# xiph/daala

Hardware: AMD Instinct MI355X
Metric: 1080p all-intra transform blocks/s (filter+DCT+PVQ) (higher is better)
Workload: dtype int32 (lifting DCT/filters) + f64 (PVQ search)

## Files before the change

### daala_amd/csrc/od_occupancy.cuh

```cuda
#pragma once
#ifndef ODHIP_SEARCH_OCC
# define ODHIP_SEARCH_OCC 0
#endif
#if ODHIP_SEARCH_OCC == 2
# define OD_SEARCH_OCC_ATTR __attribute__((amdgpu_waves_per_eu(2), amdgpu_num_vgpr(100)))
# define OD_SEARCH_VGPR_FLOOR() asm volatile("" ::: "v175")
#elif ODHIP_SEARCH_OCC == 3
# define OD_SEARCH_OCC_ATTR __attribute__((amdgpu_waves_per_eu(3), amdgpu_num_vgpr(68)))
# define OD_SEARCH_VGPR_FLOOR() asm volatile("" ::: "v128")
#else
# define OD_SEARCH_OCC_ATTR __attribute__((amdgpu_waves_per_eu(3)))
# define OD_DECIDE_OCC_ATTR
# define OD_SEARCH_VGPR_FLOOR() ((void)0)
#endif
#ifndef OD_DECIDE_OCC_ATTR
# define OD_DECIDE_OCC_ATTR OD_SEARCH_OCC_ATTR
#endif
#ifndef ODHIP_SEARCH_WAVES
# define ODHIP_SEARCH_WAVES 1
#endif
```

### daala_amd/csrc/pvq_lane.cuh

```cuda
#pragma once
#include "od_sel.cuh"

namespace {

constexpr int kPitch = 64;
constexpr int kRsqN = 512;

__device__ double gRsqTable[kRsqN];

__global__ void k_rsq_fill(void) {
  const int i = threadIdx.x;
  if (i < kRsqN) {
    gRsqTable[i] = i < 16 ? kRsqrtTable[i] : __ddiv_rn(1., __dsqrt_rn((double)(i + 1)));
  }
}

struct LaneSearch {
  double xx;
  double norm2;
  double l1_inv;
  unsigned xmax;
  unsigned xy;
  unsigned yy;
  int i;
// ... 74 lines not shown
  unsigned xmax = 0;
#pragma unroll 8
  for (int j = 0; j < N; j++) {
    const unsigned ax = pk[j*kPitch + lane] >> 16;
    xx += (unsigned long long)ax*ax;
    l1 += ax;
    xmax = ax > xmax ? ax : xmax;
  }
  xx = od_grp_add<S>(xx);
  l1 = od_grp_add<S>(l1);
  xmax = od_grp_umax<S>(xmax);
  s.xx = (double)xx;
  s.norm2 = 2*__ddiv_rn(1., __dsqrt_rn(1e-30 + s.xx));
  const double l1d = (double)l1;
  s.l1_inv = __ddiv_rn(1., l1d > 1e-100 ? l1d : 1e-100);
  s.xmax = xmax;
  s.xy = 0;
  s.yy = 0;
  s.i = 0;
}

constexpr int kGrp = 8;

template <int N>
__device__ __forceinline__ void od_lane_load_group(uint32_t (&w)[kGrp], const uint32_t *pk, int lane,
 int g) {
#pragma unroll
  for (int t = 0; t < kGrp; t++) {
    const int j = g*kGrp + t;
    w[t] = j < N ? pk[j*kPitch + lane] : 0;
  }
}

template <int N, bool ACCEL>
__device__ __forceinline__ int od_lane_rdo_scan(const uint32_t *pk, const double *rsq, int lane,
 unsigned xy, unsigned base, double norm2, double lambda, double delta_rate, double accel_rate,
 int jbase, double &best_out) {
  if (N <= 16) {
    double best = 0;
    int pos = jbase;
    int jv = jbase;
#pragma unroll 4
    for (int j = 0; j < N; j++) {
      const uint32_t w = pk[j*kPitch + lane];
      const double tt = (double)(xy + (w >> 16));
      const double r = rsq[base + (w & 0xffffu)];
      if (j > 0) od_inc(jv);
      const double jd = (double)jv;
      const double val = (tt*norm2)*r - (lambda*jd)*(ACCEL ? delta_rate + jd*accel_rate : delta_rate);
      if (j == 0) best = val;
      else {
        const unsigned long long m = od_cmp_gt(val, best);
        best = od_sel(m, val, best);
        pos = od_sel(m, jv, pos);
      }
    }
    best_out = best;
    return pos;
  }
  constexpr int NG = (N + kGrp - 1)/kGrp;
  uint32_t w0[kGrp];
  uint32_t w1[kGrp];
  uint32_t w2[kGrp];
  double r0[kGrp];
  double r1[kGrp];
  od_lane_load_group<N>(w0, pk, lane, 0);
  od_lane_load_group<N>(w1, pk, lane, 1);
#pragma unroll
  for (int t = 0; t < kGrp; t++) r0[t] = rsq[base + (w0[t] & 0xffffu)];
  double best = 0;
  int pos = jbase;
  int jv = jbase;
#pragma unroll
  for (int g = 0; g < NG; g++) {
    if (g + 2 < NG) od_lane_load_group<N>(w2, pk, lane, g + 2);
    if (g + 1 < NG) {
#pragma unroll
      for (int t = 0; t < kGrp; t++) r1[t] = rsq[base + (w1[t] & 0xffffu)];
    }
    __builtin_amdgcn_sched_barrier(0);
#pragma unroll
    for (int t = 0; t < kGrp; t++) {
      const int j = g*kGrp + t;
      if (j < N) {
        const double tt = (double)(xy + (w0[t] >> 16));
        if (j > 0) od_inc(jv);
        const double jd = (double)jv;
        const double val = (tt*norm2)*r0[t]
         - (lambda*jd)*(ACCEL ? delta_rate + jd*accel_rate : delta_rate);
        if (j == 0) best = val;
        else {
          const unsigned long long m = od_cmp_gt(val, best);
          best = od_sel(m, val, best);
          pos = od_sel(m, jv, pos);
        }
      }
    }
    __builtin_amdgcn_sched_barrier(0);
#pragma unroll
    for (int t = 0; t < kGrp; t++) {
      w0[t] = w1[t];
      w1[t] = w2[t];
      r0[t] = r1[t];
    }
  }
  best_out = best;
  return pos;
}

template <int N>
__device__ __forceinline__ int od_lane_greedy_scan(const uint32_t *pk, int lane, unsigned xy,
 unsigned yyp1, int jbase, double &ba_out, double &bb_out) {
  if (N <= 16) {
    double ba = 0;
    double bb = 1;
    int pos = jbase;
    int jv = jbase;
#pragma unroll 4
    for (int j = 0; j < N; j++) {
      const uint32_t w = pk[j*kPitch + lane];
      const double tt = (double)(xy + (w >> 16));
      const double a = tt*tt;
      const double b = (double)(yyp1 + (w & 0xffffu));
      if (j == 0) {
        ba = a;
        bb = b;
      }
      else {
        od_inc(jv);
        const unsigned long long m = od_cmp_gt(a*bb, ba*b);
        ba = od_sel(m, a, ba);
        bb = od_sel(m, b, bb);
        pos = od_sel(m, jv, pos);
      }
    }
    ba_out = ba;
    bb_out = bb;
    return pos;
  }
  constexpr int NG = (N + kGrp - 1)/kGrp;
  uint32_t w0[kGrp];
  uint32_t w1[kGrp];
  od_lane_load_group<N>(w0, pk, lane, 0);
  double ba = 0;
  double bb = 1;
  int pos = jbase;
  int jv = jbase;
#pragma unroll
  for (int g = 0; g < NG; g++) {
    if (g + 1 < NG) od_lane_load_group<N>(w1, pk, lane, g + 1);
    __builtin_amdgcn_sched_barrier(0);
#pragma unroll
    for (int t = 0; t < kGrp; t++) {
      const int j = g*kGrp + t;
      if (j < N) {
        const double tt = (double)(xy + (w0[t] >> 16));
        const double a = tt*tt;
        const double b = (double)(yyp1 + (w0[t] & 0xffffu));
        if (j == 0) {
          ba = a;
          bb = b;
        }
        else {
          od_inc(jv);
          const unsigned long long m = od_cmp_gt(a*bb, ba*b);
          ba = od_sel(m, a, ba);
          bb = od_sel(m, b, bb);
          pos = od_sel(m, jv, pos);
        }
      }
    }
    __builtin_amdgcn_sched_barrier(0);
#pragma unroll
    for (int t = 0; t < kGrp; t++) w0[t] = w1[t];
  }
  ba_out = ba;
  bb_out = bb;
  return pos;
}

#ifndef ODHIP_GREEDY_FRONTS
# define ODHIP_GREEDY_FRONTS 1
#endif
#ifndef ODHIP_FRONT_CLASSES
# define ODHIP_FRONT_CLASSES 8
#endif
#ifndef ODHIP_FRONT_MIN
# define ODHIP_FRONT_MIN 4
#endif
constexpr int kFrontClasses = ODHIP_FRONT_CLASSES;
constexpr int kFrontMinPulses = ODHIP_FRONT_MIN;

template <int N>
__device__ __forceinline__ uint32_t od_lane_front_scan(const uint32_t *pk, int lane, uint32_t c2) {
  static_assert(N % kGrp == 0, "whole groups");
  constexpr int NG = N/kGrp;
  uint32_t best = 0;
  uint32_t w0[kGrp];
// ... 68 lines not shown
    const double oa = od_pair_swap(ba);
    const double ob = od_pair_swap(bb);
    const int op = od_pair_swap(bpos);
    const int oc = od_pair_swap(bc);
    const bool ohave = od_pair_swap((int)have) != 0;
    const double l = oa*bb;
    const double r = ba*ob;
    const bool other = ohave && (!have || l > r || (l == r && op < bpos));
    const int pos = other ? op : bpos;
    const int cw = other ? oc : bc;
    const bool owner = pos/N == half;
    const int local = pos - jbase;
    uint32_t w = 0;
    if (step && owner) w = pk[local*kPitch + lane];
    w = od_grp_or<2>(w);
    const bool mine = step && owner;
    if (step) {
      s.xy += w >> 16;
      s.yy += (w & 0xffffu) + 1;
      if (owner) pk[local*kPitch + lane] = w + 2;
      s.i++;
    }
    const uint32_t nf = od_lane_front_scan<N>(pk, lane, mine ? 2u*(uint32_t)cw : 0xffffffffu);
    const uint32_t wkey = ((w + 2) & 0xffff0000u) + (0x10000u + (uint32_t)(N - 1 - local));
#pragma unroll
    for (int c = 0; c < kFrontClasses; c++) {
      if (mine && c == cw) fr[c] = nf;
      if (mine && c == cw + 1) fr[c] = wkey > fr[c] ? wkey : fr[c];
    }
    if (__any(mine && cw + 1 >= kFrontClasses)) return;
  }
}

template <int N, int S>
__device__ __forceinline__ double od_lane_search(LaneSearch &s, uint32_t *pk, const double *rsq,
 int lane, int half, bool on, bool fresh, int k, double g2, double pvq_norm_lambda,
 bool force_seq) {
  constexpr int NBAND = N*S;
  static_assert(S == 1 || S == 2 || S == 4, "one lane, a pair or a quad per band");
  const int jbase = S > 1 ? half*N : 0;
  fresh = fresh && on;
  if (__any(fresh)) {
    const double kd = fresh && k > 2 ? (double)k : 0.;
    unsigned xy = 0;
    unsigned yy = 0;
    int i = 0;
#pragma unroll 4
    for (int j = 0; j < N; j++) {
      const unsigned ax = pk[j*kPitch + lane] >> 16;
      const double tmp = (kd*(double)ax)*s.l1_inv;
      int yj = (int)floor(tmp);
      yj = yj > 0 ? yj : 0;
      if (fresh) pk[j*kPitch + lane] = ax << 16 | (unsigned)yj << 1;
      xy += ax*(unsigned)yj;
      yy += (unsigned)yj*(unsigned)yj;
      i += yj;
    }
    xy = od_grp_add<S>(xy);
    yy = od_grp_add<S>(yy);
    i = od_grp_add<S>(i);
    if (fresh) {
      s.xy = xy;
      s.yy = yy;
      s.i = i;
    }
  }
  const int rdo_pulses = 1 + k/4;
  const int n_greedy = k - rdo_pulses;
#if ODHIP_GREEDY_FRONTS
  if constexpr (S == 2 && N >= 32 && N % kGrp == 0) {
    if (!force_seq && __any(on && n_greedy - s.i >= kFrontMinPulses)) {
      od_lane_greedy_fronts<N>(s, pk, lane, half & 1, on, k, n_greedy);
    }
  }
#endif
  while (__any(on && s.i < n_greedy)) {
    const bool step = on && s.i < n_greedy;
    double ba;
    double bb;
    int pos = od_lane_greedy_scan<N>(pk, lane, s.xy, s.yy + 1, jbase, ba, bb);
    if constexpr (S > 1) {
      const double tmax = (double)(s.xy + s.xmax);
      const bool exact = !force_seq
       && (tmax*tmax)*(double)(s.yy + 2*(unsigned)k + 1) < 4503599627370496.;
      if (__any(step && !exact)) {
        double ra = od_grp_bcast<S, 0>(ba);
        double rb = od_grp_bcast<S, 0>(bb);
        int rp = od_grp_bcast<S, 0>(pos);
        auto rescan = [&](double &xa, double &xb, int &xp) {
#pragma unroll 1
          for (int j = 0; j < N; j++) {
            const uint32_t w = pk[j*kPitch + lane];
            const double tt = (double)(s.xy + (w >> 16));
            const double a = tt*tt;
            const double b = (double)(s.yy + 1 + (w & 0xffffu));
            if (a*xb > xa*b) {
              xa = a;
              xb = b;
              xp = jbase + j;
            }
          }
        };
        {
          double ta = ra;
          double tb = rb;
          int tp = rp;
          rescan(ta, tb, tp);
          ra = od_grp_bcast<S, 1>(ta);
          rb = od_grp_bcast<S, 1>(tb);
          rp = od_grp_bcast<S, 1>(tp);
        }
        if constexpr (S == 4) {
          double ta = ra;
          double tb = rb;
          int tp = rp;
          rescan(ta, tb, tp);
          ra = od_grp_bcast<4, 2>(ta);
          rb = od_grp_bcast<4, 2>(tb);
          rp = od_grp_bcast<4, 2>(tp);
          ta = ra;
          tb = rb;
          tp = rp;
          rescan(ta, tb, tp);
          rp = od_grp_bcast<4, 3>(tp);
        }
        pos = rp;
      }
      else {
        {
// ... 14 lines not shown
        }
        if constexpr (S == 4) {
          const double oa = od_quad_swap2(ba);
          const double ob = od_quad_swap2(bb);
          const int op = od_quad_swap2(pos);
          const bool up = (half & 2) != 0;
          const double la = up ? oa : ba;
          const double lb = up ? ob : bb;
          const int lp = up ? op : pos;
          const double xa = up ? ba : oa;
          const double xb = up ? bb : ob;
          const int xp = up ? pos : op;
          pos = xa*lb > la*xb ? xp : lp;
        }
      }
    }
    int owner = 1;
    int local = pos;
    if constexpr (S > 1) {
      owner = pos/N == half;
      local = pos - jbase;
    }
    uint32_t w = 0;
    if (step && owner) w = pk[local*kPitch + lane];
    w = od_grp_or<S>(w);
    if (step) {
      s.xy += w >> 16;
      s.yy += (w & 0xffffu) + 1;
      if (owner) pk[local*kPitch + lane] = w + 2;
      s.i++;
    }
  }
  const double lambda = __ddiv_rn(pvq_norm_lambda, 1e-30 + g2);
  double delta_rate = 3./NBAND;
  double accel_rate = 0.;
  if (k == 1) {
    if (NBAND == 15) {
      accel_rate = -8./NBAND;
      delta_rate = 4.5/NBAND - accel_rate;
    }
    else if (NBAND == 8) {
      accel_rate = 5.7/NBAND;
      delta_rate = 9.3/NBAND - accel_rate;
    }
  }
  while (__any(on && s.i < k)) {
    const bool step = on && s.i < k;
    int pos = 0;
    double best = 0;
    if (!__any(step && s.yy + 2*(unsigned)k + 1 > (unsigned)kRsqN)) {
      const unsigned base = step ? s.yy : 0;
      const unsigned xy = step ? s.xy : 0;
      if ((NBAND == 8 || NBAND == 15) && __any(step && k == 1)) {
        pos = od_lane_rdo_scan<N, true>(pk, rsq, lane, xy, base, s.norm2, lambda, delta_rate,
         accel_rate, jbase, best);
      }
      else {
        pos = od_lane_rdo_scan<N, false>(pk, rsq, lane, xy, base, s.norm2, lambda, delta_rate,
         accel_rate, jbase, best);
      }
    }
    else {
#pragma unroll 1
      for (int j = 0; j < N; j++) {
        const uint32_t w = pk[j*kPitch + lane];
        const double t = (double)(s.xy + (w >> 16));
        const unsigned idx = s.yy + (w & 0xffffu) + 1;
        double r;
        if (step && idx <= (unsigned)kRsqN) r = rsq[idx - 1];
        else r = od_rsqrt_beyond((int)(idx ? idx : 1));
        const int jg = jbase + j;
        const double val = (t*s.norm2)*r - (lambda*jg)*(delta_rate + jg*accel_rate);
        if (j == 0 || val > best) {
          best = val;
          pos = jg;
        }
      }
    }
    if constexpr (S > 1) {
      {
        const double ob = od_pair_swap(best);
        const int op = od_pair_swap(pos);
        const bool up = (half & 1) != 0;
        const double va = up ? ob : best;
        const double vb = up ? best : ob;
        const int pa = up ? op : pos;
        const int pb = up ? pos : op;
        const bool win = vb > va;
        best = win ? vb : va;
        pos = win ? pb : pa;
      }
      if constexpr (S == 4) {
        const double ob = od_quad_swap2(best);
        const int op = od_quad_swap2(pos);
        const bool up = (half & 2) != 0;
        const double va = up ? ob : best;
        const double vb = up ? best : ob;
        const int pa = up ? op : pos;
        const int pb = up ? pos : op;
        pos = vb > va ? pb : pa;
      }
    }
    int owner = 1;
    int local = pos;
    if constexpr (S > 1) {
      owner = pos/N == half;
// ... 17 lines not shown
```

### daala_amd/csrc/pvq_refbands.hip

```cpp
#include "../../include/daala_hip.h"
#include <math.h>
#include <stdio.h>
#include <stdlib.h>
#include <string.h>
#include "od_ctx.cuh"
#include "od_pvq_math.cuh"
#include "od_occupancy.cuh"
#include "od_krange.cuh"
#include "od_band_stage.cuh"
#include "gen/od_scan_tables.h"
#define OD_RSQ_TABLE_N 512
#define OD_RSQ_HUGE
#include "pvq_search.cuh"
#include "pvq_row.cuh"
#include "pvq_regs.cuh"

namespace {

constexpr int kMaxJobs = 8;
constexpr int kMaxItems = kMaxJobs*ODHIP_MAX_BANDS;
constexpr int kSlots = ODHIP_PVQ_REF_SLOTS;
constexpr int kUncCap = 1 << 16;
constexpr double kDefaultMargin = 1e-9;

struct RJob {
  const od_coeff *coef;
  const od_coeff *ref;
  const int16_t *qm;
  const int16_t *qm_inv;
  odhip_pvq_refband *rec;
  void *items;
  int16_t *y;
  int16_t *r16;
  int16_t *x16;
  int16_t *xr;
  const double *rate;
  int32_t *choice;
  od_coeff *dq;
  unsigned short *keys;
  unsigned *ids;
  unsigned *krange;
  long nblocks;
  int nplanes;
  int w;
  int h;
  int bs;
  int nb_bands;
  int len;
// ... 1271 lines not shown
      ax[i] = abs(t);
      sg |= (unsigned)(t < 0) << i;
      y[i] = 0;
    }
    if (pad) {
      ax[N - 1] = 0;
      sg &= ~(1u << (N - 1));
    }
    od_regs_norm<N>(ax, &xx, &norm_1);
  }
  __device__ __forceinline__ double search(int n_true, int k, int prev_k, double g2, double lambda) {
    return od_pvq_search_regs<N>(ax, y, n_true, k, prev_k, g2, lambda, xx, norm_1, &cxy, &cyy);
  }
  __device__ __forceinline__ int moment() const {
    int m = 0;
#pragma unroll
    for (int i = 1; i < N; i++) m += i*y[i];
    return m;
  }
  __device__ __forceinline__ void store(int16_t *dst) {
    uint4 *p = reinterpret_cast<uint4 *>(dst - SH);
    int t[N + SH];
    if (SH) t[0] = 0;
#pragma unroll
    for (int i = 0; i < N; i++) t[i + SH] = (sg >> i) & 1 ? -y[i] : y[i];
#pragma unroll
    for (int q = 0; q < (N + SH)/8; q++) {
      p[q] = make_uint4(pack16(t[8*q], t[8*q + 1]), pack16(t[8*q + 2], t[8*q + 3]),
       pack16(t[8*q + 4], t[8*q + 5]), pack16(t[8*q + 6], t[8*q + 7]));
    }
  }
};



__device__ __forceinline__ int neg_interleave(int x, int ref) {
  if (x < ref) return -2*(x - ref) - 1;
  if (x < 2*ref) return 2*(x - ref);
  return x - 1;
}

__device__ unsigned char gRBandOf[OD_SCAN_LEN];

template <int N, class YGet>
__device__ __forceinline__ void refb_finish(const RItems &it, int job, const RJob &jb, int band, long blk,
 const odhip_pvq_refband &r, const RefBest &best, YGet yget);

template <int N, int PRICE>
__device__ __forceinline__ void refb_choose_band(const RItems &it, int job, const RJob &jb, int band,
 long blk, const double *given) {
  constexpr int SH = N == 15 ? 1 : 0;
  constexpr int NW = (N + SH)/2;
  const long bi = blk*jb.nb_bands + band;
  const odhip_pvq_refband r = jb.rec[bi];
  const ItemPtr ip = item_ptr(jb, band, blk);
  const double *rate = PRICE == 2 ? given : PRICE == 0 && jb.rate ? jb.rate + bi*(kSlots + 1) : nullptr;
  const double lambda = it.lambda;
  const int off = jb.off[band];
  double best_cost = r.dist0 + lambda*(rate ? rate[0] : 0.);
  bool close = false;
  int noref = jb.is_keyframe ? 1 : 0;
  int32_t best_qtheta = 0;
  int chosen = -1;
  int yslot = -1;
  int4 tails[kSlots];
  int dlo[kSlots];
  int dhi[kSlots];
// ... 439 lines not shown
    }
  }
  if (cl.nitems > cl.ntheta) {
    v.load(jb.x16 + blk*len + off, false);
    int prev_k = 0;
    int idx = cl.ntheta;
    while (idx < cl.nitems) {
      const uint32_t w = cl.col[idx*cl.stride];
      const int i = cl.gbn + (int)(w & 3u);
#ifdef ODHIP_EXPERIMENTS
      const int k = dec.abl & 8 ? 0 : (int)(w >> 2 & 0xffffu);
#else
      const int k = (int)(w >> 2 & 0xffffu);
#endif
      const int32_t qcg = odq_shl32(i, ODQ_CGAIN_SHIFT);
      double dist = (1.4*(qcg - cg))*(qcg - cg);
      dist *= s2;
      const bool skip = (dist > dist0 && k != 0) || k > ODHIP_PVQ_MAX_K;
      const bool others = __any(skip);
      if (!skip && others) continue;
      idx++;
      if (skip) continue;
      const double cos_dist = v.search(n, k, prev_k, (qcg*(double)cg)*s2, lambda);
      prev_k = k;
      const double prate = lean_rate_pulses<NR>(v.moment(), k);
      dist = (1.4*(qcg - cg))*(qcg - cg) + (qcg*(double)cg)*(2 - 2*cos_dist);
      dist *= s2;
      dec.offer(idx - 1, false, i, -1, 0, k, 0, dist, prate, 0., true, v);
    }
  }
}

constexpr int kPreWords = 6;

template <int NR, int G, class V, class D>
__device__ __forceinline__ void refb_loops_lean_rows(const RJob &jb, int band, long blk,
 const odhip_pvq_refband &r, const CandList &cl, double lambda, V &v, D &dec, uint32_t *pre, int pre_stride) {
  const int off = jb.off[band];
  const int n = jb.off[band + 1] - off;
  const int len = jb.len;
  const double s2 = (1./256)*(1./256);
  const double t1 = 1./32768;
  const int32_t cg = r.cg;
  const double dist0 = r.dist0;
  const int32_t theta = r.theta;
  for (int c = v.l; c < kSlots; c += G) {
    if (c < cl.ntheta) {
      const uint32_t w = cl.col[c*cl.stride];
      const int gi = (int)(w & 3u);
      const int k = (int)(w >> 2 & 0xffffu);
      const int i = cl.gb1 + gi;
      const int ts = (int)cl.col[(kSlots + gi)*cl.stride];
      const int j = (int)cl.col[(kSlots + 3 + gi)*cl.stride] + (int)(w >> 18);
      const int32_t qcg = odq_shl32(i, ODQ_CGAIN_SHIFT) + r.gain_offset;
      const int32_t qtheta = odq_pvq_compute_theta(j, ts);
      const double cosfix = 2 - (2.*odq_pvq_cos(theta - qtheta))*t1;
      double dist = (1.4*(qcg - cg))*(qcg - cg) + (qcg*(double)cg)*cosfix;
      dist *= s2;
      const bool skip = (dist > dist0 + 1.0*lambda && k != 0) || k > ODHIP_PVQ_MAX_K;
      const double sin_prod = ((odq_pvq_sin(theta)*t1)*odq_pvq_sin(qtheta))*t1;
      uint32_t *p = pre + c*kPreWords*pre_stride;
      p[0] = (uint32_t)qcg;
      p[pre_stride] = skip;
      p[2*pre_stride] = (uint32_t)__double2loint(cosfix);
      p[3*pre_stride] = (uint32_t)__double2hiint(cosfix);
      p[4*pre_stride] = (uint32_t)__double2loint(sin_prod);
      p[5*pre_stride] = (uint32_t)__double2hiint(sin_prod);
    }
  }
  if constexpr (kSearchWaves == 1) __syncthreads();
  else {
    __builtin_amdgcn_fence(__ATOMIC_RELEASE, "wavefront");
    __builtin_amdgcn_wave_barrier();
    __builtin_amdgcn_fence(__ATOMIC_ACQUIRE, "wavefront");
  }
  if (cl.ntheta > 0) {
    v.load(jb.xr + blk*len + off, true);
    int prev_k = 0;
    bool has = false;
    double cos_dist = 0;
    double prate = 0;
    int idx = 0;
    while (idx < cl.ntheta) {
      const uint32_t w = cl.col[idx*cl.stride];
      const int k = (int)(w >> 2 & 0xffffu);
      const uint32_t *p = pre + idx*kPreWords*pre_stride;
      const bool skip = p[pre_stride] != 0;
      const bool want = !skip && k != 0 && k != prev_k;
      const bool others = __any(!want);
      if (want && others) continue;
      idx++;
      if (skip) continue;
      const int gi = (int)(w & 3u);
      const int i = cl.gb1 + gi;
      const int ts = (int)cl.col[(kSlots + gi)*cl.stride];
      const int j = (int)cl.col[(kSlots + 3 + gi)*cl.stride] + (int)(w >> 18);
      const int32_t qcg = (int32_t)p[0];
      const double cosfix = __hiloint2double((int)p[3*pre_stride], (int)p[2*pre_stride]);
      const double sin_prod = __hiloint2double((int)p[5*pre_stride], (int)p[4*pre_stride]);
      if (k == 0) {
        cos_dist = 0;
        has = false;
        prate = 0;
      }
      else if (want) {
        cos_dist = v.search(n - 1, k, prev_k, ((qcg*(double)cg)*sin_prod)*s2, lambda);
        has = true;
        prate = lean_rate_pulses<NR>(v.moment(), k);
      }
      prev_k = k;
      const double dist_theta = cosfix + sin_prod*(2 - 2*cos_dist);
      double dist = (1.4*(qcg - cg))*(qcg - cg) + (qcg*(double)cg)*dist_theta;
      dist *= s2;
      const double lts = __hiloint2double((int)cl.col[(kSlots + 7 + 2*gi)*cl.stride],
       (int)cl.col[(kSlots + 6 + 2*gi)*cl.stride]);
      dec.offer(idx - 1, true, i, j, ts, k, 0, dist, prate, lts, has, v);
    }
  }
  if (cl.nitems > cl.ntheta) {
    v.load(jb.x16 + blk*len + off, false);
    int prev_k = 0;
    int idx = cl.ntheta;
    while (idx < cl.nitems) {
      const uint32_t w = cl.col[idx*cl.stride];
      const int i = cl.gbn + (int)(w & 3u);
      const int k = (int)(w >> 2 & 0xffffu);
      const int32_t qcg = odq_shl32(i, ODQ_CGAIN_SHIFT);
      double dist = (1.4*(qcg - cg))*(qcg - cg);
      dist *= s2;
      const bool skip = (dist > dist0 && k != 0) || k > ODHIP_PVQ_MAX_K;
      const bool others = __any(skip);
      if (!skip && others) continue;
      idx++;
      if (skip) continue;
      const double cos_dist = v.search(n, k, prev_k, (qcg*(double)cg)*s2, lambda);
      prev_k = k;
      const double prate = lean_rate_pulses<NR>(v.moment(), k);
      dist = (1.4*(qcg - cg))*(qcg - cg) + (qcg*(double)cg)*(2 - 2*cos_dist);
      dist *= s2;
      dec.offer(idx - 1, false, i, -1, 0, k, 0, dist, prate, 0., true, v);
    }
  }
}

template <int NY>
struct LeanDecide {
  double best_cost;
  int chosen;
  bool close;
  int y[NY];
  unsigned sg;
  double lambda;
  double tol_scale;
  int icgr;
  int is_keyframe;
  int pli;
#ifdef ODHIP_EXPERIMENTS
  int abl = 0;
#endif
// ... 80 lines not shown
  const RJob &jb = it.jobs[job];
  const long pos = (long)(unit - it.wg_start[item])*kWave + lane;
  if (pos >= jb.nblocks) return;
  const int band = it.band[item];
  const long blk = jb.ids[(long)band*jb.nblocks + pos];
  const odhip_pvq_refband r = jb.rec[blk*jb.nb_bands + band];
  const CandList cl = refb_build_list(jb, band, r, s_list + lane, kWave, true);
  RegVector<N> v;
  LeanDecide<N> dec;
  dec.init(r, jb, it.lambda, it.tol_scale);
#ifdef ODHIP_EXPERIMENTS
  dec.abl = it.abl;
#endif
  refb_loops_lean_gathered<N>(jb, band, blk, r, cl, it.lambda, v, dec);
  const RefBest best = lean_best(dec, cl, jb.is_keyframe);
  if (best.yslot >= 0) {
    uint4 *p = reinterpret_cast<uint4 *>(jb.y + blk*jb.len + jb.off[band] - SH);
    int t[N + SH];
    if (SH) t[0] = 0;
#pragma unroll
    for (int i = 0; i < N; i++) t[i + SH] = dec.signed_y(i);
#pragma unroll
    for (int q = 0; q < (N + SH)/8; q++) {
      p[q] = make_uint4(pack16(t[8*q], t[8*q + 1]), pack16(t[8*q + 2], t[8*q + 3]),
       pack16(t[8*q + 4], t[8*q + 5]), pack16(t[8*q + 6], t[8*q + 7]));
    }
  }
  refb_finish<N>(it, job, jb, band, blk, r, best, [&](int i) -> int { return dec.signed_y(i); });
}

template <int G>
__device__ __forceinline__ int grp_from_prev(int v, int l) {
  if (G == 16) return __builtin_amdgcn_update_dpp(0, v, 0x111 , 0xf, 0xf, true);
  const int t = row_mov<0x90>(v);
  return l == 0 ? 0 : t;
}

template <int E, int G>
__device__ __forceinline__ void refb_finish_row(const RItems &it, int job, const RJob &jb, int band, long blk,
 const odhip_pvq_refband &r, const LeanDecide<E> &dec, const RefBest &best, int l, bool live) {
  constexpr int n = G*E;
  const long bi = blk*jb.nb_bands + band;
  const int off = jb.off[band];
  const int cfl_enabled = jb.is_keyframe && jb.pli != 0;
  const bool writer = live && l == 0;
  const int chosen = best.chosen;
  const int yslot = best.yslot;
  const int noref = best.noref;
  int qg = 0;
  int itheta = jb.is_keyframe ? -1 : 0;
  int max_theta = 0;
  int best_k = 0;
  if (best.close && writer) {
    const unsigned slot = atomicAdd(it.pcount, 1u);
    if (slot < (unsigned)kPUncCap) {
      PUncR *e = it.plist + slot;
      e->job = job;
      e->band = band;
      e->blk = (unsigned)blk;
    }
  }
  if (chosen >= 0) {
    qg = best.gain;
    best_k = best.k;
    if (!noref) {
      itheta = best.theta;
      max_theta = best.ts;
    }
    else {
      itheta = -1;
      max_theta = 0;
    }
  }
  int skip = 0;
  if (noref) {
    if (qg == 0) skip = 1;
  }
  else {
    if (!jb.is_keyframe && qg == 0) skip = r.icgr ? 1 : 2;
    if (qg == r.icgr && itheta == 0 && !cfl_enabled) skip = 2;
  }
  int4 *ch = reinterpret_cast<int4 *>(jb.choice + bi*16);
  if (writer) {
    ch[0] = make_int4(chosen, qg, noref, itheta);
    ch[1] = make_int4(max_theta, best_k, skip, jb.is_keyframe ? (noref ? qg : neg_interleave(qg, r.icgr))
     : (noref ? qg - 1 : neg_interleave(qg + 1, r.icgr + 1)));
  }
  if (skip) {
    if (writer) {
      const int flip = (r.flags & ODHIP_REFBAND_FLIP) != 0;
      ch[2] = make_int4(skip == 2 ? (flip ? 4 : 1) : 0, -1, 0, 0);
      ch[3] = make_int4(0, 0, 0, 0);
    }
    return;
  }
  int wy[E];
#pragma unroll
  for (int e = 0; e < E; e++) wy[e] = dec.signed_y(e);
  if (live && yslot >= 0) {
    int16_t *p = jb.y + blk*jb.len + off + l*E;
    static_assert(E == 8, "one 16-byte piece per lane");
    *reinterpret_cast<uint4 *>(p) = make_uint4(pack16(wy[0], wy[1]), pack16(wy[2], wy[3]), pack16(wy[4], wy[5]),
     pack16(wy[6], wy[7]));
  }
  const int32_t g = odq_gain_expand(odq_shl32(qg, ODQ_CGAIN_SHIFT) + (noref ? 0 : r.gain_offset),
   job_q(jb, band, blk), jb.beta[band]);
  int yy = 0;
#pragma unroll
  for (int e = 0; e < E; e++) yy += wy[e]*wy[e];
  yy = grp_sum<G>(yy);
  int gshift = odq_ilog(g) - 14;
  gshift = gshift > 0 ? gshift : 0;
  int32_t scale = 0;
  if (yy != 0) {
    int rsqrt_shift;
    const int16_t rsqrt = odq_rsqrt(yy, &rsqrt_shift);
    scale = odq_vshr_round(rsqrt*(int64_t)g, rsqrt_shift + gshift - 16);
  }
  const int qshift = ODQ_QM_INV_SHIFT - gshift;
  if (noref) {
    if (writer) {
      ch[2] = make_int4(2, yslot, scale, qshift);
      ch[3] = make_int4(0, 0, 0, 0);
    }
    return;
  }
  const int m = r.m;
  const int s = r.s;
  scale = (int32_t)floor(.5 + (scale*(1./32768))*odq_pvq_sin(best.qtheta));
  const int16_t xm = (int16_t)floor(.5 + ((-s*odq_shr_round(g, gshift))*(1./32768))*odq_pvq_cos(best.qtheta));
  const uint4 r4 = *reinterpret_cast<const uint4 *>(jb.r16 + blk*jb.len + off + l*E);
  const uint32_t rw[4] = {r4.x, r4.y, r4.z, r4.w};
  const int yprev = grp_from_prev<G>(wy[E - 1], l);
  int32_t l2r = 0;
  int32_t proj = 0;
#pragma unroll
  for (int e = 0; e < E; e++) {
    const int i = l*E + e;
    const int ri = (int16_t)(rw[e >> 1] >> (16*(e & 1)));
    const int ysrc = i < m ? wy[e] : (e == 0 ? yprev : wy[e > 0 ? e - 1 : 0]);
    const int16_t xi = i == m ? xm : (int16_t)odq_mult16_32_q16(ysrc, scale);
    l2r += odq_mult16_16(ri, ri);
    proj += odq_mult16_16(ri, xi);
  }
  l2r = grp_sum<G>(l2r);
  proj = grp_sum<G>(proj);
  int16_t proj_1;
  int outshift;
  householder_consts(l2r, proj, &proj_1, &outshift);
  if (writer) {
    ch[2] = make_int4(3, yslot, scale, qshift);
    ch[3] = make_int4(xm, m, proj_1, outshift);
  }
  (void)n;
}

template <int E, int G>
__global__ __launch_bounds__(kSearchThreads) OD_SEARCH_OCC_ATTR void k_refb_lean_row(RItems it) {
  constexpr int C = kWave/G;
  __shared__ uint32_t s_list_w[kSearchWaves][kLeanWords*C];
  __shared__ uint32_t s_pre_w[kSearchWaves][kSlots*kPreWords*C];
  OD_SEARCH_VGPR_FLOOR();
  od_rsqrt_init(threadIdx.x);
  const int wave = __builtin_amdgcn_readfirstlane(threadIdx.x/kWave);
  const int unit = blockIdx.x*kSearchWaves + wave;
  if (unit >= it.wg_start[it.nitems]) return;
  uint32_t *s_list = s_list_w[wave];
  uint32_t *s_pre = s_pre_w[wave];
  const int item = find_item(it, unit);
  const int job = it.job[item];
  const RJob &jb = it.jobs[job];
  const int band = it.band[item];
  const int lane = threadIdx.x%kWave;
  RowVector<E, G> v;
  v.row = lane/G;
  v.l = lane%G;
  v.force = it.perturb >> 1;
  const long nblocks = jb.nblocks;
  const long pos = (long)(unit - it.wg_start[item])*C + v.row;
  const bool live = pos < nblocks;
  const long blk = jb.ids[(long)band*nblocks + (live ? pos : nblocks - 1)];
  const odhip_pvq_refband r = jb.rec[blk*jb.nb_bands + band];
  const CandList cl = refb_build_list(jb, band, r, s_list + v.row, C, v.l == 0);
  LeanDecide<E> dec;
  dec.init(r, jb, it.lambda, it.tol_scale);
  refb_loops_lean_rows<G*E, G>(jb, band, blk, r, cl, it.lambda, v, dec, s_pre + v.row, C);
  refb_finish_row<E, G>(it, job, jb, band, blk, r, dec, lean_best(dec, cl, jb.is_keyframe), v.l, live);
#ifdef ODHIP_EXPERIMENTS
  if (live && v.l == 0) {
    if (v.pulses) atomicAdd(&gRowReplayStats[0], (unsigned long long)v.pulses);
    if (v.replays) atomicAdd(&gRowReplayStats[1], (unsigned long long)v.replays);
    if (v.rate_pulses) atomicAdd(&gRowReplayStats[2], (unsigned long long)v.rate_pulses);
    atomicAdd(&gRowReplayStats[3], 1ull);
  }
#endif
}

template <int N>
__global__ __launch_bounds__(kWave) void k_refb_choose_unc_list(RItems it, const Unc *list, int count) {
  const int i = blockIdx.x*kWave + threadIdx.x;
  if (i >= count) return;
  const Unc e = list[i];
  const RJob &jb = it.jobs[e.job];
  if (jb.off[e.band + 1] - jb.off[e.band] != N) return;
  refb_choose_band<N, 1>(it, e.job, jb, e.band, e.blk, nullptr);
}

template <int N, int PRICE>
__global__ __launch_bounds__(kWave) void k_refb_choose(RItems it) {
  const int item = find_item(it, blockIdx.x);
  const int job = it.job[item];
  const RJob &jb = it.jobs[job];
  const long blk = (long)(blockIdx.x - it.wg_start[item])*kWave + threadIdx.x;
  if (blk >= jb.nblocks) return;
  refb_choose_band<N, PRICE>(it, job, jb, it.band[item], blk, nullptr);
}

template <int N>
__global__ __launch_bounds__(kWave) void k_refb_choose_list(RItems it, const PUncR *list, int count) {
  const int i = blockIdx.x*kWave + threadIdx.x;
  if (i >= count) return;
  const PUncR *e = list + i;
  const RJob &jb = it.jobs[e->job];
  if (jb.off[e->band + 1] - jb.off[e->band] != N) return;
  refb_choose_band<N, 2>(it, e->job, jb, e->band, e->blk, e->rate);
}

__global__ __launch_bounds__(256) void k_refb_synth(RItems it) {
// ... 300 lines not shown
  RItems pi;
  const auto prep = [&](void (*kernel)(RItems), int size, long per_wg) {
    items_begin(pi, st, lambda);
    pi.fuse = stage;
    if (size) items_add_size(pi, host, njobs, size, per_wg, 1);
    else for (int j = 0; j < njobs; j++) items_add(pi, j, 0, (host[j].nblocks + per_wg - 1)/per_wg);
    if (pi.nitems) kernel<<<pi.wg_start[pi.nitems], kWave, 0, s>>>(pi);
  };
#ifdef ODHIP_EXPERIMENTS
  static const bool split = getenv("ODHIP_REFB_PREP_SPLIT") != nullptr;
  if (split) {
    prep(k_refb_prep_lane<15>, 0, kWave);
    prep(k_refb_prep_lane<8>, 8, kWave);
  }
  else
#endif
  prep(k_refb_prep_corner, 0, kWave);
  prep(k_refb_prep_row<8, 4>, 32, 16);
  prep(k_refb_prep_row<8, 16>, 128, 4);
}

int sort_blocks(RefState &st, const RJob *host, int njobs, hipStream_t s) {
  return st.sort.run(host, st.tabs.cur, njobs, s);
}

struct RefSearch {
  int size;
  int on;
  int per_wg;
  bool row;
};
constexpr RefSearch kRefSearches[4] = {{128, 0, 4, true}, {32, 1, 16, true}, {15, 2, kWave, false},
 {8, 2, kWave, false}};

void launch_search(RefState &st, RItems &it, const RefSearch &r, RefStage stage, hipStream_t s) {
  if (stage == kStageDecided) items_heavy_first(it);
  const int wgs = it.wg_start[it.nitems];
  const int groups = (wgs + kSearchWaves - 1)/kSearchWaves;
  const auto regs = [&](auto priced) {
    for_band_size(r.size, [&](auto size) {
      constexpr int N = decltype(size)::value;
      if constexpr (N <= 15) k_refb_search_regs<N, decltype(priced)::value><<<wgs, kWave, 0, s>>>(it);
    });
  };
  const auto launch = [&] {
    if (r.row) {
      for_band_size(r.size, [&](auto size) {
        constexpr int N = decltype(size)::value;
        if constexpr (N >= 32) {
          if (stage == kStageDecided) k_refb_lean_row<8, N/8><<<groups, kSearchThreads, 0, s>>>(it);
          else k_refb_search_row<8, N/8><<<wgs, kWave, 0, s>>>(it);
        }
      });
    }
    else if (stage == kStageDecided) {
      for_band_size(r.size, [&](auto size) {
        constexpr int N = decltype(size)::value;
        if constexpr (N <= 15) k_refb_lean_lane<N><<<groups, kSearchThreads, 0, s>>>(it);
      });
    }
    else if (stage == kStageLanePriced) regs(std::true_type());
    else regs(std::false_type());
  };
  if (r.size == 128) st.prof.around(s, launch);
  else launch();
}

int launch_searches(RefState &st, const RJob *host, int njobs, double lambda, RefStage stage, hipStream_t s) {
  const bool lane_only = stage != kStageDecided && ODHIP_EXP_ENV("ODHIP_PVQ_REF_LANE") != nullptr;
  hipStream_t side[2] = {s, s};
  if (st.streams.fork(s, side) != ODHIP_SUCCESS) return ODHIP_EFAULT;
  const hipStream_t streams[3] = {s, side[0], side[1]};
  RItems it;
  for (const RefSearch &r : kRefSearches) {
    items_begin(it, st, lambda);
    if (r.row && !lane_only && odhip_env_force_seq()) it.perturb |= 2;
    items_add_size(it, host, njobs, r.size, lane_only ? kWave : r.per_wg);
    if (it.nitems && !lane_only) launch_search(st, it, r, stage, streams[r.on]);
#ifdef ODHIP_EXPERIMENTS
    if (it.nitems && lane_only) {
      k_refb_search<<<it.wg_start[it.nitems], kWave, (size_t)2*r.size*kWave*sizeof(unsigned short), streams[r.on]>>>(it);
    }
#endif
  }
  if (st.streams.join(s, side) != ODHIP_SUCCESS) return ODHIP_EFAULT;
  return ODHIP_SUCCESS;
}

int ref_bands(const odhip_pvq_refjob *jobs, int njobs, double pvq_norm_lambda, odhip_stream stream, RefStage stage) {
  hipStream_t s = (hipStream_t)stream;
  REF_STATE_OR_RETURN(st);
  RJob host[kMaxJobs];
  int rc = stage_jobs(st, jobs, njobs, kJobBands, host, s);
  if (rc) return rc;
  ODHIP_TRY(hipMemsetAsync(st.unc_count(), 0, (stage != kStageRecords ? 2 : 1)*sizeof(unsigned), s));
  st.lean = stage == kStageDecided;
  RItems it;
  items_begin(it, st, pvq_norm_lambda);
  items_add_size(it, host, njobs, 0, kWave);
  if (!it.nitems) return ODHIP_SUCCESS;
  launch_prep(st, host, njobs, pvq_norm_lambda, stage, s);
  if (stage != kStageDecided) k_refb_cands<<<it.wg_start[it.nitems], kWave, 0, s>>>(it);
  rc = sort_blocks(st, host, njobs, s);
  if (rc) return rc;
  rc = launch_searches(st, host, njobs, pvq_norm_lambda, stage, s);
  if (rc) return rc;
  if (stage == kStageDecided) {
    rc = st.unc_posted.post(st.unc_count(), s);
    if (!rc) rc = st.priced.post(st.pcount(), s);
    if (rc) return rc;
// ... 284 lines not shown
```

Baseline: 1.174 billion.

## Search size-32 decided bands with lane pairs per band instead of row groups

```diff
diff --git a/daala_amd/csrc/od_occupancy.cuh b/daala_amd/csrc/od_occupancy.cuh
--- a/daala_amd/csrc/od_occupancy.cuh
+++ b/daala_amd/csrc/od_occupancy.cuh
@@ -19,3 +19,13 @@
 #ifndef ODHIP_SEARCH_WAVES
 # define ODHIP_SEARCH_WAVES 1
 #endif
+#ifndef ODHIP_PAIR_WAVES
+# define ODHIP_PAIR_WAVES 8
+#endif
+#ifndef OD_PAIR_OCC_ATTR
+# if ODHIP_SEARCH_OCC == 0
+#  define OD_PAIR_OCC_ATTR __attribute__((amdgpu_waves_per_eu(4)))
+# else
+#  define OD_PAIR_OCC_ATTR OD_SEARCH_OCC_ATTR
+# endif
+#endif
diff --git a/daala_amd/csrc/pvq_lane.cuh b/daala_amd/csrc/pvq_lane.cuh
--- a/daala_amd/csrc/pvq_lane.cuh
+++ b/daala_amd/csrc/pvq_lane.cuh
@@ -130,10 +130,11 @@
   }
 }
 
-template <int N, bool ACCEL>
+template <int N, bool ACCEL, bool PAD = false>
 __device__ __forceinline__ int od_lane_rdo_scan(const uint32_t *pk, const double *rsq, int lane,
  unsigned xy, unsigned base, double norm2, double lambda, double delta_rate, double accel_rate,
- int jbase, double &best_out) {
+ int jbase, double &best_out, unsigned long long keep = ~0ull) {
+  static_assert(!PAD || N > 1, "the PAD is the lane's last position and never its first");
   if (N <= 16) {
     double best = 0;
     int pos = jbase;
@@ -148,7 +149,8 @@
       const double val = (tt*norm2)*r - (lambda*jd)*(ACCEL ? delta_rate + jd*accel_rate : delta_rate);
       if (j == 0) best = val;
       else {
-        const unsigned long long m = od_cmp_gt(val, best);
+        unsigned long long m = od_cmp_gt(val, best);
+        if (PAD && j == N - 1) m &= keep;
         best = od_sel(m, val, best);
         pos = od_sel(m, jv, pos);
       }
@@ -188,7 +190,8 @@
          - (lambda*jd)*(ACCEL ? delta_rate + jd*accel_rate : delta_rate);
         if (j == 0) best = val;
         else {
-          const unsigned long long m = od_cmp_gt(val, best);
+          unsigned long long m = od_cmp_gt(val, best);
+          if (PAD && j == N - 1) m &= keep;
           best = od_sel(m, val, best);
           pos = od_sel(m, jv, pos);
         }
@@ -206,9 +209,10 @@
   return pos;
 }
 
-template <int N>
+template <int N, bool PAD = false>
 __device__ __forceinline__ int od_lane_greedy_scan(const uint32_t *pk, int lane, unsigned xy,
- unsigned yyp1, int jbase, double &ba_out, double &bb_out) {
+ unsigned yyp1, int jbase, double &ba_out, double &bb_out, unsigned long long keep = ~0ull) {
+  static_assert(!PAD || N > 1, "the PAD is the lane's last position and never its first");
   if (N <= 16) {
     double ba = 0;
     double bb = 1;
@@ -226,7 +230,8 @@
       }
       else {
         od_inc(jv);
-        const unsigned long long m = od_cmp_gt(a*bb, ba*b);
+        unsigned long long m = od_cmp_gt(a*bb, ba*b);
+        if (PAD && j == N - 1) m &= keep;
         ba = od_sel(m, a, ba);
         bb = od_sel(m, b, bb);
         pos = od_sel(m, jv, pos);
@@ -261,7 +266,8 @@
         }
         else {
           od_inc(jv);
-          const unsigned long long m = od_cmp_gt(a*bb, ba*b);
+          unsigned long long m = od_cmp_gt(a*bb, ba*b);
+          if (PAD && j == N - 1) m &= keep;
           ba = od_sel(m, a, ba);
           bb = od_sel(m, b, bb);
           pos = od_sel(m, jv, pos);
@@ -396,13 +402,17 @@
   }
 }
 
-template <int N, int S>
+template <int N, int S, bool PAD = false>
 __device__ __forceinline__ double od_lane_search(LaneSearch &s, uint32_t *pk, const double *rsq,
  int lane, int half, bool on, bool fresh, int k, double g2, double pvq_norm_lambda,
- bool force_seq) {
+ bool force_seq, bool pad = false) {
   constexpr int NBAND = N*S;
   static_assert(S == 1 || S == 2 || S == 4, "one lane, a pair or a quad per band");
+  static_assert(!PAD || (NBAND - 1 != 8 && NBAND - 1 != 15 && NBAND != 8 && NBAND != 15),
+   "the k == 1 special cases of the short bands are not formed for a padded search");
   const int jbase = S > 1 ? half*N : 0;
+  const bool pad_lane = PAD && pad && half == S - 1;
+  const unsigned long long keep = PAD ? ~__ballot(pad_lane) : ~0ull;
   fresh = fresh && on;
   if (__any(fresh)) {
     const double kd = fresh && k > 2 ? (double)k : 0.;
@@ -432,7 +442,7 @@
   const int rdo_pulses = 1 + k/4;
   const int n_greedy = k - rdo_pulses;
 #if ODHIP_GREEDY_FRONTS
-  if constexpr (S == 2 && N >= 32 && N % kGrp == 0) {
+  if constexpr (!PAD && S == 2 && N >= 32 && N % kGrp == 0) {
     if (!force_seq && __any(on && n_greedy - s.i >= kFrontMinPulses)) {
       od_lane_greedy_fronts<N>(s, pk, lane, half & 1, on, k, n_greedy);
     }
@@ -442,7 +452,7 @@
     const bool step = on && s.i < n_greedy;
     double ba;
     double bb;
-    int pos = od_lane_greedy_scan<N>(pk, lane, s.xy, s.yy + 1, jbase, ba, bb);
+    int pos = od_lane_greedy_scan<N, PAD>(pk, lane, s.xy, s.yy + 1, jbase, ba, bb, keep);
     if constexpr (S > 1) {
       const double tmax = (double)(s.xy + s.xmax);
       const bool exact = !force_seq
@@ -458,7 +468,7 @@
             const double tt = (double)(s.xy + (w >> 16));
             const double a = tt*tt;
             const double b = (double)(s.yy + 1 + (w & 0xffffu));
-            if (a*xb > xa*b) {
+            if (a*xb > xa*b && !(PAD && pad_lane && j == N - 1)) {
               xa = a;
               xb = b;
               xp = jbase + j;
@@ -539,7 +549,7 @@
     }
   }
   const double lambda = __ddiv_rn(pvq_norm_lambda, 1e-30 + g2);
-  double delta_rate = 3./NBAND;
+  double delta_rate = PAD && pad ? 3./(NBAND - 1) : 3./NBAND;
   double accel_rate = 0.;
   if (k == 1) {
     if (NBAND == 15) {
@@ -559,12 +569,12 @@
       const unsigned base = step ? s.yy : 0;
       const unsigned xy = step ? s.xy : 0;
       if ((NBAND == 8 || NBAND == 15) && __any(step && k == 1)) {
-        pos = od_lane_rdo_scan<N, true>(pk, rsq, lane, xy, base, s.norm2, lambda, delta_rate,
-         accel_rate, jbase, best);
+        pos = od_lane_rdo_scan<N, true, PAD>(pk, rsq, lane, xy, base, s.norm2, lambda, delta_rate,
+         accel_rate, jbase, best, keep);
       }
       else {
-        pos = od_lane_rdo_scan<N, false>(pk, rsq, lane, xy, base, s.norm2, lambda, delta_rate,
-         accel_rate, jbase, best);
+        pos = od_lane_rdo_scan<N, false, PAD>(pk, rsq, lane, xy, base, s.norm2, lambda, delta_rate,
+         accel_rate, jbase, best, keep);
       }
     }
     else {
@@ -578,7 +588,7 @@
         else r = od_rsqrt_beyond((int)(idx ? idx : 1));
         const int jg = jbase + j;
         const double val = (t*s.norm2)*r - (lambda*jg)*(delta_rate + jg*accel_rate);
-        if (j == 0 || val > best) {
+        if (j == 0 || (val > best && !(PAD && pad_lane && j == N - 1))) {
           best = val;
           pos = jg;
         }
diff --git a/daala_amd/csrc/pvq_refbands.hip b/daala_amd/csrc/pvq_refbands.hip
--- a/daala_amd/csrc/pvq_refbands.hip
+++ b/daala_amd/csrc/pvq_refbands.hip
@@ -14,6 +14,7 @@
 #include "pvq_search.cuh"
 #include "pvq_row.cuh"
 #include "pvq_regs.cuh"
+#include "pvq_lane.cuh"
 
 namespace {
 
@@ -1351,7 +1352,57 @@
   }
 };
 
-
+template <int NL>
+struct PairVector {
+  struct Pulses {
+    const uint32_t *col;
+    __device__ __forceinline__ int operator[](int e) const { return (int)(col[e*kPitch] >> 1 & 0x7fffu); }
+  };
+  uint32_t *pk;
+  Pulses y;
+  unsigned sg;
+  int lane;
+  int l;
+  bool force_seq;
+  LaneSearch st;
+  __device__ __forceinline__ void init(uint32_t *columns, int lane_in, bool force) {
+    pk = columns;
+    y.col = columns + lane_in;
+    lane = lane_in;
+    l = lane_in & 1;
+    force_seq = force;
+  }
+  __device__ __forceinline__ void load(const int16_t *src, bool pad) {
+    static_assert(NL % 8 == 0, "whole 16-byte pieces");
+    const uint4 *p = reinterpret_cast<const uint4 *>(src + l*NL);
+    sg = 0;
+#pragma unroll
+    for (int q = 0; q < NL/8; q++) {
+      const uint4 t = p[q];
+      const uint32_t w[4] = {t.x, t.y, t.z, t.w};
+#pragma unroll
+      for (int e = 0; e < 8; e++) {
+        const int j = 8*q + e;
+        int v = (int16_t)(w[e >> 1] >> (16*(e & 1)));
+        if (j == NL - 1 && pad && l == 1) v = 0;
+        pk[j*kPitch + lane] = (uint32_t)abs(v) << 16;
+        sg |= (unsigned)(v < 0) << j;
+      }
+    }
+    od_lane_prepare<NL, 2>(st, pk, lane);
+  }
+  __device__ __forceinline__ double search(int n_true, int k, int prev_k, double g2, double lambda) {
+    const bool fresh = !(prev_k > 0 && prev_k <= k);
+    return od_lane_search<NL, 2, true>(st, pk, od_rsq_lds, lane, l, true, fresh, k, g2, lambda, force_seq,
+     n_true != 2*NL);
+  }
+  __device__ __forceinline__ int moment() const {
+    int m = 0;
+#pragma unroll
+    for (int e = 0; e < NL; e++) m += (l*NL + e)*y[e];
+    return od_grp_add<2>(m);
+  }
+};
 
 __device__ __forceinline__ int neg_interleave(int x, int ref) {
   if (x < ref) return -2*(x - ref) - 1;
@@ -1857,8 +1908,9 @@
 }
 
 constexpr int kPreWords = 6;
-
-template <int NR, int G, class V, class D>
+constexpr int kPrePacked = 1;
+
+template <int NR, int G, class V, class D, bool PACKED = false, int WAVES = kSearchWaves>
 __device__ __forceinline__ void refb_loops_lean_rows(const RJob &jb, int band, long blk,
  const odhip_pvq_refband &r, const CandList &cl, double lambda, V &v, D &dec, uint32_t *pre, int pre_stride) {
   const int off = jb.off[band];
@@ -1869,6 +1921,7 @@
   const int32_t cg = r.cg;
   const double dist0 = r.dist0;
   const int32_t theta = r.theta;
+  uint32_t skips = 0;
   for (int c = v.l; c < kSlots; c += G) {
     if (c < cl.ntheta) {
       const uint32_t w = cl.col[c*cl.stride];
@@ -1879,21 +1932,30 @@
       const int j = (int)cl.col[(kSlots + 3 + gi)*cl.stride] + (int)(w >> 18);
       const int32_t qcg = odq_shl32(i, ODQ_CGAIN_SHIFT) + r.gain_offset;
       const int32_t qtheta = odq_pvq_compute_theta(j, ts);
-      const double cosfix = 2 - (2.*odq_pvq_cos(theta - qtheta))*t1;
+      const int cosd = odq_pvq_cos(theta - qtheta);
+      const double cosfix = 2 - (2.*cosd)*t1;
       double dist = (1.4*(qcg - cg))*(qcg - cg) + (qcg*(double)cg)*cosfix;
       dist *= s2;
       const bool skip = (dist > dist0 + 1.0*lambda && k != 0) || k > ODHIP_PVQ_MAX_K;
-      const double sin_prod = ((odq_pvq_sin(theta)*t1)*odq_pvq_sin(qtheta))*t1;
-      uint32_t *p = pre + c*kPreWords*pre_stride;
-      p[0] = (uint32_t)qcg;
-      p[pre_stride] = skip;
-      p[2*pre_stride] = (uint32_t)__double2loint(cosfix);
-      p[3*pre_stride] = (uint32_t)__double2hiint(cosfix);
-      p[4*pre_stride] = (uint32_t)__double2loint(sin_prod);
-      p[5*pre_stride] = (uint32_t)__double2hiint(sin_prod);
-    }
-  }
-  if constexpr (kSearchWaves == 1) __syncthreads();
+      if constexpr (PACKED) {
+        skips |= (uint32_t)skip << c;
+        pre[c*kPrePacked*pre_stride] = ((uint32_t)cosd & 0xffffu) | (uint32_t)odq_pvq_sin(qtheta) << 16;
+      }
+      else {
+        const double sin_prod = ((odq_pvq_sin(theta)*t1)*odq_pvq_sin(qtheta))*t1;
+        uint32_t *p = pre + c*kPreWords*pre_stride;
+        p[0] = (uint32_t)qcg;
+        p[pre_stride] = skip;
+        p[2*pre_stride] = (uint32_t)__double2loint(cosfix);
+        p[3*pre_stride] = (uint32_t)__double2hiint(cosfix);
+        p[4*pre_stride] = (uint32_t)__double2loint(sin_prod);
+        p[5*pre_stride] = (uint32_t)__double2hiint(sin_prod);
+      }
+    }
+  }
+  static_assert(!PACKED || (G == 2 && kSlots <= 32), "the two halves of a pair's skip mask");
+  if constexpr (PACKED) skips = od_grp_or<2>(skips);
+  if constexpr (WAVES == 1) __syncthreads();
   else {
     __builtin_amdgcn_fence(__ATOMIC_RELEASE, "wavefront");
     __builtin_amdgcn_wave_barrier();
@@ -1908,9 +1970,13 @@
     int idx = 0;
     while (idx < cl.ntheta) {
       const uint32_t w = cl.col[idx*cl.stride];
+#ifdef ODHIP_EXPERIMENTS
+      const int k = dec.abl & 8 ? 0 : (int)(w >> 2 & 0xffffu);
+#else
       const int k = (int)(w >> 2 & 0xffffu);
-      const uint32_t *p = pre + idx*kPreWords*pre_stride;
-      const bool skip = p[pre_stride] != 0;
+#endif
+      const uint32_t *p = pre + idx*(PACKED ? kPrePacked : kPreWords)*pre_stride;
+      const bool skip = PACKED ? (skips >> idx & 1u) != 0 : p[pre_stride] != 0;
       const bool want = !skip && k != 0 && k != prev_k;
       const bool others = __any(!want);
       if (want && others) continue;
@@ -1920,9 +1986,20 @@
       const int i = cl.gb1 + gi;
       const int ts = (int)cl.col[(kSlots + gi)*cl.stride];
       const int j = (int)cl.col[(kSlots + 3 + gi)*cl.stride] + (int)(w >> 18);
-      const int32_t qcg = (int32_t)p[0];
-      const double cosfix = __hiloint2double((int)p[3*pre_stride], (int)p[2*pre_stride]);
-      const double sin_prod = __hiloint2double((int)p[5*pre_stride], (int)p[4*pre_stride]);
+      int32_t qcg;
+      double cosfix;
+      double sin_prod;
+      if constexpr (PACKED) {
+        const uint32_t cs = p[0];
+        qcg = odq_shl32(i, ODQ_CGAIN_SHIFT) + r.gain_offset;
+        cosfix = 2 - (2.*(int16_t)(cs & 0xffffu))*t1;
+        sin_prod = ((odq_pvq_sin(theta)*t1)*(int16_t)(cs >> 16))*t1;
+      }
+      else {
+        qcg = (int32_t)p[0];
+        cosfix = __hiloint2double((int)p[3*pre_stride], (int)p[2*pre_stride]);
+        sin_prod = __hiloint2double((int)p[5*pre_stride], (int)p[4*pre_stride]);
+      }
       if (k == 0) {
         cos_dist = 0;
         has = false;
@@ -1949,7 +2026,11 @@
     while (idx < cl.nitems) {
       const uint32_t w = cl.col[idx*cl.stride];
       const int i = cl.gbn + (int)(w & 3u);
+#ifdef ODHIP_EXPERIMENTS
+      const int k = dec.abl & 8 ? 0 : (int)(w >> 2 & 0xffffu);
+#else
       const int k = (int)(w >> 2 & 0xffffu);
+#endif
       const int32_t qcg = odq_shl32(i, ODQ_CGAIN_SHIFT);
       double dist = (1.4*(qcg - cg))*(qcg - cg);
       dist *= s2;
@@ -2096,8 +2177,14 @@
 template <int G>
 __device__ __forceinline__ int grp_from_prev(int v, int l) {
   if (G == 16) return __builtin_amdgcn_update_dpp(0, v, 0x111 , 0xf, 0xf, true);
-  const int t = row_mov<0x90>(v);
+  const int t = G == 2 ? od_pair_swap(v) : row_mov<0x90>(v);
   return l == 0 ? 0 : t;
+}
+
+template <int G>
+__device__ __forceinline__ int grp_total(int v) {
+  if constexpr (G == 2) return od_grp_add<2>(v);
+  else return grp_sum<G>(v);
 }
 
 template <int E, int G>
@@ -2162,17 +2249,20 @@
 #pragma unroll
   for (int e = 0; e < E; e++) wy[e] = dec.signed_y(e);
   if (live && yslot >= 0) {
-    int16_t *p = jb.y + blk*jb.len + off + l*E;
-    static_assert(E == 8, "one 16-byte piece per lane");
-    *reinterpret_cast<uint4 *>(p) = make_uint4(pack16(wy[0], wy[1]), pack16(wy[2], wy[3]), pack16(wy[4], wy[5]),
-     pack16(wy[6], wy[7]));
+    uint4 *p = reinterpret_cast<uint4 *>(jb.y + blk*jb.len + off + l*E);
+    static_assert(E % 8 == 0, "whole 16-byte pieces per lane");
+#pragma unroll
+    for (int q = 0; q < E/8; q++) {
+      p[q] = make_uint4(pack16(wy[8*q], wy[8*q + 1]), pack16(wy[8*q + 2], wy[8*q + 3]),
+       pack16(wy[8*q + 4], wy[8*q + 5]), pack16(wy[8*q + 6], wy[8*q + 7]));
+    }
   }
   const int32_t g = odq_gain_expand(odq_shl32(qg, ODQ_CGAIN_SHIFT) + (noref ? 0 : r.gain_offset),
    job_q(jb, band, blk), jb.beta[band]);
   int yy = 0;
 #pragma unroll
   for (int e = 0; e < E; e++) yy += wy[e]*wy[e];
-  yy = grp_sum<G>(yy);
+  yy = grp_total<G>(yy);
   int gshift = odq_ilog(g) - 14;
   gshift = gshift > 0 ? gshift : 0;
   int32_t scale = 0;
@@ -2193,8 +2283,15 @@
   const int s = r.s;
   scale = (int32_t)floor(.5 + (scale*(1./32768))*odq_pvq_sin(best.qtheta));
   const int16_t xm = (int16_t)floor(.5 + ((-s*odq_shr_round(g, gshift))*(1./32768))*odq_pvq_cos(best.qtheta));
-  const uint4 r4 = *reinterpret_cast<const uint4 *>(jb.r16 + blk*jb.len + off + l*E);
-  const uint32_t rw[4] = {r4.x, r4.y, r4.z, r4.w};
+  uint32_t rw[E/2];
+#pragma unroll
+  for (int q = 0; q < E/8; q++) {
+    const uint4 r4 = reinterpret_cast<const uint4 *>(jb.r16 + blk*jb.len + off + l*E)[q];
+    rw[4*q] = r4.x;
+    rw[4*q + 1] = r4.y;
+    rw[4*q + 2] = r4.z;
+    rw[4*q + 3] = r4.w;
+  }
   const int yprev = grp_from_prev<G>(wy[E - 1], l);
   int32_t l2r = 0;
   int32_t proj = 0;
@@ -2207,8 +2304,8 @@
     l2r += odq_mult16_16(ri, ri);
     proj += odq_mult16_16(ri, xi);
   }
-  l2r = grp_sum<G>(l2r);
-  proj = grp_sum<G>(proj);
+  l2r = grp_total<G>(l2r);
+  proj = grp_total<G>(proj);
   int16_t proj_1;
   int outshift;
   householder_consts(l2r, proj, &proj_1, &outshift);
@@ -2248,6 +2345,9 @@
   const CandList cl = refb_build_list(jb, band, r, s_list + v.row, C, v.l == 0);
   LeanDecide<E> dec;
   dec.init(r, jb, it.lambda, it.tol_scale);
+#ifdef ODHIP_EXPERIMENTS
+  dec.abl = it.abl;
+#endif
   refb_loops_lean_rows<G*E, G>(jb, band, blk, r, cl, it.lambda, v, dec, s_pre + v.row, C);
   refb_finish_row<E, G>(it, job, jb, band, blk, r, dec, lean_best(dec, cl, jb.is_keyframe), v.l, live);
 #ifdef ODHIP_EXPERIMENTS
@@ -2258,6 +2358,48 @@
     atomicAdd(&gRowReplayStats[3], 1ull);
   }
 #endif
+}
+
+constexpr int kPairWaves = ODHIP_PAIR_WAVES;
+constexpr int kPairThreads = kPairWaves*kWave;
+
+template <int NL>
+__global__ __launch_bounds__(kPairThreads) OD_PAIR_OCC_ATTR void k_refb_lean_pair(RItems it) {
+  constexpr int G = 2;
+  constexpr int C = kWave/G;
+  static_assert(kRsqN == OD_RSQ_TABLE_N && kPitch == kWave, "od_lane_search on this unit's table and columns");
+  __shared__ uint32_t s_list_w[kPairWaves][kLeanWords*C];
+  __shared__ uint32_t s_pre_w[kPairWaves][kSlots*kPrePacked*C];
+  __shared__ uint32_t s_pk_w[kPairWaves][NL*kPitch];
+  OD_SEARCH_VGPR_FLOOR();
+  od_rsqrt_init(threadIdx.x);
+  const int wave = __builtin_amdgcn_readfirstlane(threadIdx.x/kWave);
+  const int unit = blockIdx.x*kPairWaves + wave;
+  if (unit >= it.wg_start[it.nitems]) return;
+  uint32_t *s_list = s_list_w[wave];
+  uint32_t *s_pre = s_pre_w[wave];
+  const int item = find_item(it, unit);
+  const int job = it.job[item];
+  const RJob &jb = it.jobs[job];
+  const int band = it.band[item];
+  const int lane = threadIdx.x%kWave;
+  const int row = lane/G;
+  PairVector<NL> v;
+  v.init(s_pk_w[wave], lane, (it.perturb >> 1) != 0);
+  const long nblocks = jb.nblocks;
+  const long pos = (long)(unit - it.wg_start[item])*C + row;
+  const bool live = pos < nblocks;
+  const long blk = jb.ids[(long)band*nblocks + (live ? pos : nblocks - 1)];
+  const odhip_pvq_refband r = jb.rec[blk*jb.nb_bands + band];
+  const CandList cl = refb_build_list(jb, band, r, s_list + row, C, v.l == 0);
+  LeanDecide<NL> dec;
+  dec.init(r, jb, it.lambda, it.tol_scale);
+#ifdef ODHIP_EXPERIMENTS
+  dec.abl = it.abl;
+#endif
+  refb_loops_lean_rows<G*NL, G, PairVector<NL>, LeanDecide<NL>, true, kPairWaves>(jb, band, blk, r, cl,
+   it.lambda, v, dec, s_pre + row, C);
+  refb_finish_row<NL, G>(it, job, jb, band, blk, r, dec, lean_best(dec, cl, jb.is_keyframe), v.l, live);
 }
 
 template <int N>
@@ -2624,6 +2766,12 @@
 };
 constexpr RefSearch kRefSearches[4] = {{128, 0, 4, true}, {32, 1, 16, true}, {15, 2, kWave, false},
  {8, 2, kWave, false}};
+constexpr int kPairBands = kWave/2;
+
+bool pair_search(const RefSearch &r, RefStage stage) {
+  static const bool row32 = ODHIP_EXP_ENV("ODHIP_REFB_ROW32") != nullptr;
+  return r.size == 32 && stage == kStageDecided && !row32;
+}
 
 void launch_search(RefState &st, RItems &it, const RefSearch &r, RefStage stage, hipStream_t s) {
   if (stage == kStageDecided) items_heavy_first(it);
@@ -2636,7 +2784,8 @@
     });
   };
   const auto launch = [&] {
-    if (r.row) {
+    if (pair_search(r, stage)) k_refb_lean_pair<16><<<(wgs + kPairWaves - 1)/kPairWaves, kPairThreads, 0, s>>>(it);
+    else if (r.row) {
       for_band_size(r.size, [&](auto size) {
         constexpr int N = decltype(size)::value;
         if constexpr (N >= 32) {
@@ -2667,7 +2816,7 @@
   for (const RefSearch &r : kRefSearches) {
     items_begin(it, st, lambda);
     if (r.row && !lane_only && odhip_env_force_seq()) it.perturb |= 2;
-    items_add_size(it, host, njobs, r.size, lane_only ? kWave : r.per_wg);
+    items_add_size(it, host, njobs, r.size, lane_only ? kWave : pair_search(r, stage) ? kPairBands : r.per_wg);
     if (it.nitems && !lane_only) launch_search(st, it, r, stage, streams[r.on]);
 #ifdef ODHIP_EXPERIMENTS
     if (it.nitems && lane_only) {
```

New measurement: 1.226 billion (median of 6 runs). 4.4% higher.
